# AlerianEmperor/Voxel-Cone-Tracing

Hardware: AMD Instinct MI355X
Metric: Mcones/s (+ ms per GI pass), Sponza-class 256^3 @1080p (higher is better)
Workload: dtype f32; 1 GPU; procedural atrium (Sponza-class, 257488 tris, seed 1234), 256^3 RGBA8 brick chain, 1920x1080, 6 diffuse + 1 specular cone/px, trace of a resident (GPU-rasterised) G-buffer; voxel_dim=256, width=1920, height=1080, cones_per_pixel=7, bounces=1, anisotropic_mips=False, parallelism=single GPU, trace_variant=0, footprint_records=False, comm_reserved_cus=0, raster_form=direct

## Files before the change

### voxel-cone-tracing_amd/csrc/vct_trace.hip

```cpp
#include <hip/hip_fp16.h>

#include <type_traits>

#include "../../include/vct.h"
#include "vct_internal.h"
#include "vct_texel.h"
#include "vct_tilediv.h"


namespace {

struct F3 { float x, y, z; };
struct F4 { float x, y, z, w; };

__device__ __forceinline__ F3 f3(float x, float y, float z) { return {x, y, z}; }
__device__ __forceinline__ float dot3(F3 a, F3 b) { return a.x * b.x + a.y * b.y + a.z * b.z; }
__device__ __forceinline__ F3 cross3(F3 a, F3 b) {
    return {a.y * b.z - a.z * b.y, a.z * b.x - a.x * b.z, a.x * b.y - a.y * b.x};
}
__device__ __forceinline__ float div_rn(float a, float b) { return a / b; }
__device__ __forceinline__ float sqrt_rn(float a) { return __builtin_sqrtf(a); }
__device__ __forceinline__ F3 normalize3(F3 a) {
    const float l = sqrt_rn(dot3(a, a));
    return {div_rn(a.x, l), div_rn(a.y, l), div_rn(a.z, l)};
// ... 71 lines not shown
struct Footprint { int i0, j0, k0; float a, b, c; };
__device__ __forceinline__ Footprint footprint_of(const VctLevelRef lv, float ux, float uy, float uz) {
    const float fN = lv.fN;
    const float u = fmaf(ux, fN, -0.5f), v = fmaf(uy, fN, -0.5f), w = fmaf(uz, fN, -0.5f);
    const float fu = floorf(u), fv = floorf(v), fw = floorf(w);
    const float a = u - fu, b = v - fv, c = w - fw;
    return {(int)fu, (int)fv, (int)fw, a, b, c};
}
struct Anchor { int x, y, z; };
__device__ __forceinline__ int anchor_lane(unsigned long long am) {
    return ((am >> 27) & 1ull) ? 27 : (int)__ffsll((long long)am) - 1;
}
__device__ __forceinline__ Anchor anchor_of(const Footprint& f, int src) {
    return {__builtin_amdgcn_readlane(f.i0, src) - 1, __builtin_amdgcn_readlane(f.j0, src) - 1,
            __builtin_amdgcn_readlane(f.k0, src) - 1};
}
struct BlockFit { int dx, dy, dz; unsigned long long out; };
__device__ __forceinline__ BlockFit block_fit(const Footprint& f, const Anchor an, unsigned long long am) {
    const int dx = f.i0 - an.x, dy = f.j0 - an.y, dz = f.k0 - an.z;
    const uint32_t far = max(max((uint32_t)dx, (uint32_t)dy), (uint32_t)dz);
    return {dx, dy, dz, ballot64(far > 2u) & am};
}
template <bool WRAP>
__device__ __forceinline__ uint32_t block_texel_index(const VctLevelRef lv, const Anchor an, const LaneBlock& lb) {
    if (WRAP) {
        const uint32_t MX = lv.mask_x, MY = MX << 1, MZ = MX << 2;
        const uint32_t m4 = (uint32_t)lv.m << 2;
        const uint32_t sax = spread_byte(lb.lut, an.x, m4) >> 2;
        const uint32_t say = spread_byte(lb.lut, an.y, m4) >> 1;
        const uint32_t saz = spread_byte(lb.lut, an.z, m4);
        return (((sax | ~MX) + lb.sbx) & MX) | (((say | ~MY) + lb.sby) & MY) | (((saz | ~MZ) + lb.sbz) & MZ);
    } else {
        const int x = min(max(an.x + (lb.lane & 3), 0), lv.m);
        const int y = min(max(an.y + ((lb.lane >> 2) & 3), 0), lv.m);
        const int z = min(max(an.z + (lb.lane >> 4), 0), lv.m);
        return vct_morton3((uint32_t)x, (uint32_t)y, (uint32_t)z);
    }
}
__device__ __forceinline__ int block_slot(bool act, int dx, int dy, int dz) { return act ? (dz * 4 + dy) * 4 + dx : 0; }
__device__ __forceinline__ unsigned long long block_texel_mask(const float4 d) {
    return ballot64((__float_as_uint(d.x) | __float_as_uint(d.y) | __float_as_uint(d.z) | __float_as_uint(d.w)) != 0u);
}

#ifndef VCT_REUSE
#define VCT_REUSE 1
#endif
#define VCT_NO_BLOCK 0xfffffff0u
struct BlockDesc {
    uint32_t id;
    Anchor an;
};
__device__ __forceinline__ BlockDesc no_block() { return {VCT_NO_BLOCK, {0, 0, 0}}; }

__device__ __forceinline__ F4 gather_block(const float4* q, float a, float b, float c) {
    F4 r;
    const float a0 = 1.0f - a, b0 = 1.0f - b, c0 = 1.0f - c;
    const float ab00 = a0 * b0, ab10 = a * b0, ab01 = a0 * b, ab11 = a * b;
    {
        const float4 t0 = q[0], t1 = q[1], t2 = q[4], t3 = q[5];
        const float w0 = ab00 * c0, w1 = ab10 * c0, w2 = ab01 * c0, w3 = ab11 * c0;
#define VCT_ACC(ch) r.ch = w0 * t0.ch; r.ch = fmaf(w1, t1.ch, r.ch); r.ch = fmaf(w2, t2.ch, r.ch); r.ch = fmaf(w3, t3.ch, r.ch);
        VCT_ACC(x) VCT_ACC(y) VCT_ACC(z) VCT_ACC(w)
#undef VCT_ACC
    }
    __builtin_amdgcn_sched_barrier(0);
    {
        const float4 t4 = q[16], t5 = q[17], t6 = q[20], t7 = q[21];
        wave_sync();
        const float w4 = ab00 * c, w5 = ab10 * c, w6 = ab01 * c, w7 = ab11 * c;
#define VCT_ACC(ch) r.ch = fmaf(w4, t4.ch, r.ch); r.ch = fmaf(w5, t5.ch, r.ch); r.ch = fmaf(w6, t6.ch, r.ch); r.ch = fmaf(w7, t7.ch, r.ch);
        VCT_ACC(x) VCT_ACC(y) VCT_ACC(z) VCT_ACC(w)
#undef VCT_ACC
    }
    return r;
}

__device__ __forceinline__ void per_lane_census(MarchStats& ms, const Footprint& f, bool act, unsigned long long am, int lane) {
    const int i0 = f.i0, j0 = f.j0, k0 = f.k0;
    ++ms.fallback; ms.fallback_lanes += (uint32_t)__popcll(am);
    int lo[3] = {act ? i0 : 0x7fffffff, act ? j0 : 0x7fffffff, act ? k0 : 0x7fffffff};
    int hi[3] = {act ? i0 : -0x7fffffff, act ? j0 : -0x7fffffff, act ? k0 : -0x7fffffff};
    for (int off = 32; off > 0; off >>= 1)
        for (int q = 0; q < 3; ++q) { lo[q] = min(lo[q], __shfl_xor(lo[q], off)); hi[q] = max(hi[q], __shfl_xor(hi[q], off)); }
    if (hi[0] - lo[0] <= 2 && hi[1] - lo[1] <= 2 && hi[2] - lo[2] <= 2) ++ms.fallback_fits;
    unsigned long long pending = am;
    int nb = 0;
    while (pending != 0ull && nb < 16) {
        const BlockFit fit = block_fit(f, anchor_of(f, (int)__ffsll((long long)pending) - 1), ~0ull);
        pending &= fit.out;
        ++nb;
    }
    int qlo[3] = {act ? i0 : 0x7fffffff, act ? j0 : 0x7fffffff, act ? k0 : 0x7fffffff};
    int qhi[3] = {act ? i0 : -0x7fffffff, act ? j0 : -0x7fffffff, act ? k0 : -0x7fffffff};
    bool qany = act;
    auto widen = [&](int off) {
        for (int q = 0; q < 3; ++q) { qlo[q] = min(qlo[q], __shfl_xor(qlo[q], off)); qhi[q] = max(qhi[q], __shfl_xor(qhi[q], off)); }
        qany = qany || (__shfl_xor((int)qany, off) != 0);
    };
    widen(1); widen(8);
    const int span2 = max(max(qhi[0] - qlo[0], qhi[1] - qlo[1]), qhi[2] - qlo[2]);
    const bool lead2 = (lane & 9) == 0;
    ms.quads_live += (uint32_t)__popcll(ballot64(lead2 && qany));
    ms.quads_fit333 += (uint32_t)__popcll(ballot64(lead2 && qany && span2 <= 1));
    ms.quads_same += (uint32_t)__popcll(ballot64(lead2 && qany && span2 == 0));
    widen(2); widen(16);
    const int span4 = max(max(qhi[0] - qlo[0], qhi[1] - qlo[1]), qhi[2] - qlo[2]);
    const bool lead4 = (lane & 27) == 0;
    ms.quadrants_live += (uint32_t)__popcll(ballot64(lead4 && qany));
    ms.quadrants_fit444 += (uint32_t)__popcll(ballot64(lead4 && qany && span4 <= 2));
    ms.greedy_blocks += (uint32_t)nb;
    if (nb <= 2) ++ms.greedy_le2;
    if (nb <= 3) ++ms.greedy_le3;
    if (nb <= 4) ++ms.greedy_le4;
}

template <bool WRAP, bool COOP, bool LOOSE = false, bool CELLS = false, bool PRIO = false>
__device__ __forceinline__ F4 sample_level(const uint32_t* __restrict__ chain, const VctLevelRef lv,
                                           float ux, float uy, float uz, bool act, unsigned long long am,
                                           float4* __restrict__ blk, const LaneBlock& lb, MarchStats& ms,
                                           const char* __restrict__ cells = nullptr) {
    if (PRIO) __builtin_amdgcn_s_setprio(1);
    const int m = lv.m;
    const Footprint f = footprint_of(lv, ux, uy, uz);
    const float a = f.a, b = f.b, c = f.c;
    const int i0 = f.i0, j0 = f.j0, k0 = f.k0;
    const uint32_t* __restrict__ base = chain + lv.off;
    const uint32_t MX = lv.mask_x, MY = MX << 1, MZ = MX << 2;
    const vct_v4i32 tb = level_texel_buffer(base);

    F4 r = {0.0f, 0.0f, 0.0f, 0.0f};
    const Anchor an = anchor_of(f, anchor_lane(am));
    const BlockFit fit = block_fit(f, an, am);
    if (COOP && fit.out == 0ull) {
        const float4 d = texel_f32(tb, block_texel_index<WRAP>(lv, an, lb));
        if (PRIO) __builtin_amdgcn_s_setprio(0);
        const bool any_texel = block_texel_mask(d) != 0ull;
        if (VCT_STATS) { if (any_texel) ++ms.coop_hit; else ++ms.coop_zero; }
        if (any_texel) {
            blk[lb.lane] = d;
            wave_sync();
            r = gather_block(blk + block_slot(act, fit.dx, fit.dy, fit.dz), a, b, c);
        }
    } else {
      if (VCT_STATS) per_lane_census(ms, f, act, am, lb.lane);
      if (act) {
        uint32_t mx0, mx1, my0, my1, mz0, mz1;
        if (WRAP) {
            if (!CELLS) {
                const uint32_t m4 = (uint32_t)m << 2;
                const char* lutb = (const char*)lb.lut_vec;
                mx0 = *(const uint32_t*)(lutb + (((uint32_t)i0 << 2) & m4)) >> 2;
                my0 = *(const uint32_t*)(lutb + (((uint32_t)j0 << 2) & m4)) >> 1;
                mz0 = *(const uint32_t*)(lutb + (((uint32_t)k0 << 2) & m4));
            } else {
                mx0 = vct_spread3((uint32_t)i0 & (uint32_t)m);
                my0 = vct_spread3((uint32_t)j0 & (uint32_t)m) << 1;
                mz0 = vct_spread3((uint32_t)k0 & (uint32_t)m) << 2;
            }
            mx1 = ((mx0 | ~MX) + 1u) & MX;
            my1 = ((my0 | ~MY) + 2u) & MY;
            mz1 = ((mz0 | ~MZ) + 4u) & MZ;
        } else {
            const int ci0 = min(max(i0, 0), m), ci1 = min(max(i0 + 1, 0), m);
            const int cj0 = min(max(j0, 0), m), cj1 = min(max(j0 + 1, 0), m);
            const int ck0 = min(max(k0, 0), m), ck1 = min(max(k0 + 1, 0), m);
            mx0 = vct_spread3((uint32_t)ci0); mx1 = vct_spread3((uint32_t)ci1);
            my0 = vct_spread3((uint32_t)cj0) << 1; my1 = vct_spread3((uint32_t)cj1) << 1;
            mz0 = vct_spread3((uint32_t)ck0) << 2; mz1 = vct_spread3((uint32_t)ck1) << 2;
        }
        if (!CELLS) {
            const float a0 = 1.0f - a, b0 = 1.0f - b, c0 = 1.0f - c;
            const float ab00 = a0 * b0, ab10 = a * b0, ab01 = a0 * b, ab11 = a * b;
            {
                const float4 f0 = texel_f32(tb, mx0 | my0 | mz0), f1 = texel_f32(tb, mx1 | my0 | mz0);
                const float w0 = ab00 * c0, w1 = ab10 * c0;
#define VCT_ACC(ch) r.ch = w0 * f0.ch; r.ch = fmaf(w1, f1.ch, r.ch);
                VCT_ACC(x) VCT_ACC(y) VCT_ACC(z) VCT_ACC(w)
#undef VCT_ACC
            }
            __builtin_amdgcn_sched_barrier(0);
            {
                const float4 f2 = texel_f32(tb, mx0 | my1 | mz0), f3 = texel_f32(tb, mx1 | my1 | mz0);
                const float w2 = ab01 * c0, w3 = ab11 * c0;
#define VCT_ACC(ch) r.ch = fmaf(w2, f2.ch, r.ch); r.ch = fmaf(w3, f3.ch, r.ch);
                VCT_ACC(x) VCT_ACC(y) VCT_ACC(z) VCT_ACC(w)
#undef VCT_ACC
            }
            __builtin_amdgcn_sched_barrier(0);
            {
                const float4 f4 = texel_f32(tb, mx0 | my0 | mz1), f5 = texel_f32(tb, mx1 | my0 | mz1);
                const float4 f6 = texel_f32(tb, mx0 | my1 | mz1), f7 = texel_f32(tb, mx1 | my1 | mz1);
                if (PRIO) __builtin_amdgcn_s_setprio(0);
                const float w4 = ab00 * c, w5 = ab10 * c, w6 = ab01 * c, w7 = ab11 * c;
#define VCT_ACC(ch) r.ch = fmaf(w4, f4.ch, r.ch); r.ch = fmaf(w5, f5.ch, r.ch); r.ch = fmaf(w6, f6.ch, r.ch); r.ch = fmaf(w7, f7.ch, r.ch);
                VCT_ACC(x) VCT_ACC(y) VCT_ACC(z) VCT_ACC(w)
#undef VCT_ACC
            }
        } else {
            uint32_t t[8];
            if (WRAP && lv.off != 0u) {
                const char* cb = cells + ((size_t)lv.off << 5);
                const uint32_t ro = (mx0 | my0 | mz0) << 5;
                const uint4 lo = *(const uint4*)(cb + ro);
                const uint4 hi = *(const uint4*)(cb + ro + 16u);
                t[0] = lo.x; t[1] = lo.y; t[2] = lo.z; t[3] = lo.w;
                t[4] = hi.x; t[5] = hi.y; t[6] = hi.z; t[7] = hi.w;
            } else {
                t[0] = base[mx0 | my0 | mz0]; t[1] = base[mx1 | my0 | mz0];
                t[2] = base[mx0 | my1 | mz0]; t[3] = base[mx1 | my1 | mz0];
                t[4] = base[mx0 | my0 | mz1]; t[5] = base[mx1 | my0 | mz1];
                t[6] = base[mx0 | my1 | mz1]; t[7] = base[mx1 | my1 | mz1];
            }
            if (PRIO) __builtin_amdgcn_s_setprio(0);
            const float a0 = 1.0f - a, b0 = 1.0f - b, c0 = 1.0f - c;
            const float wg[8] = {(a0 * b0) * c0, (a * b0) * c0, (a0 * b) * c0, (a * b) * c0,
                                 (a0 * b0) * c,  (a * b0) * c,  (a0 * b) * c,  (a * b) * c};
            r.x = wg[0] * unorm8_of<0, LOOSE>(t[0]);
            r.y = wg[0] * unorm8_of<8, LOOSE>(t[0]);
            r.z = wg[0] * unorm8_of<16, LOOSE>(t[0]);
            r.w = wg[0] * unorm8_of<24, LOOSE>(t[0]);
#pragma unroll
            for (int i = 1; i < 8; ++i) {
                r.x = fmaf(wg[i], unorm8_of<0, LOOSE>(t[i]), r.x);
                r.y = fmaf(wg[i], unorm8_of<8, LOOSE>(t[i]), r.y);
                r.z = fmaf(wg[i], unorm8_of<16, LOOSE>(t[i]), r.z);
                r.w = fmaf(wg[i], unorm8_of<24, LOOSE>(t[i]), r.w);
            }
        }
      }
    }
    return r;
}

template <bool WRAP, bool LOOSE, bool PRIO, int SLAB>
__device__ __forceinline__ F4 sample_level_reuse(const uint32_t* __restrict__ chain, const VctLevelRef lv,
                                                 float ux, float uy, float uz, bool act, unsigned long long am,
                                                 float4* __restrict__ blk, const LaneBlock& lb, MarchStats& ms,
                                                 BlockDesc& held) {
    if (PRIO) __builtin_amdgcn_s_setprio(1);
    const Footprint f = footprint_of(lv, ux, uy, uz);
    int mode = 0, at = 0;
    if ((held.id & ~1u) == lv.off) {
        const BlockDesc cd = held;
        const BlockFit fit = block_fit(f, cd.an, am);
        if (VCT_STATS) {
            const Anchor fresh = anchor_of(f, anchor_lane(am));
            ++ms.reuse[SLAB][0];
            if (fit.out == 0ull) { ++ms.reuse[SLAB][1]; if (!(cd.id & 1u)) ++ms.reuse[SLAB][2]; }
            if (fresh.x == cd.an.x && fresh.y == cd.an.y && fresh.z == cd.an.z) ++ms.reuse[SLAB][3];
        }
        if (fit.out == 0ull) {
            if (PRIO) __builtin_amdgcn_s_setprio(0);
            mode = 1 + (int)(cd.id & 1u);
            at = block_slot(act, fit.dx, fit.dy, fit.dz) + 64;
        }
    }
    if (mode == 0) {
        const Anchor an = anchor_of(f, anchor_lane(am));
        const BlockFit fit = block_fit(f, an, am);
        if (fit.out == 0ull) {
            const uint32_t idx = block_texel_index<true>(lv, an, lb);
            const float4 d = texel_f32(level_texel_buffer(chain + lv.off), idx);
            if (PRIO) __builtin_amdgcn_s_setprio(0);
            const unsigned long long any_texel = block_texel_mask(d);
            if (VCT_STATS) { if (any_texel != 0ull) ++ms.coop_hit; else ++ms.coop_zero; }
            mode = any_texel != 0ull ? 2 : 1;
            if (SLAB == 1) held = {lv.off | (uint32_t)(mode - 1), an};
            if (mode == 2) {
                blk[SLAB * 64 + lb.lane] = d;
                wave_sync();
                at = block_slot(act, fit.dx, fit.dy, fit.dz) + SLAB * 64;
            }
        }
    }
    if (mode == 2) return gather_block(blk + at, f.a, f.b, f.c);
    if (mode == 1) return {0.0f, 0.0f, 0.0f, 0.0f};
    return sample_level<WRAP, false, LOOSE, false, PRIO>(chain, lv, ux, uy, uz, act, am, blk, lb, ms);
}

template <bool WRAP, bool COOP, bool LOOSE, bool CELLS, bool PRIO, bool REUSE, int SLAB>
__device__ __forceinline__ F4 sample_step_level(const VctTraceParams& p, const VctLevelRef lv, float ux, float uy, float uz,
                                                bool act, unsigned long long am, float4* __restrict__ blk,
                                                const LaneBlock& lb, MarchStats& ms, BlockDesc& held) {
    if constexpr (REUSE) {
        static_assert(WRAP && COOP && !CELLS, "block reuse: cooperative sampler, GL_REPEAT, no footprint records");
        return sample_level_reuse<WRAP, LOOSE, PRIO, SLAB>(p.chain, lv, ux, uy, uz, act, am, blk, lb, ms, held);
    } else {
        return sample_level<WRAP, COOP, LOOSE, CELLS, PRIO>(p.chain, lv, ux, uy, uz, act, am, blk + SLAB * 64, lb, ms, p.cells_biased);
    }
}

struct AnisoCone {
    float wx, wy, wz;
    bool nx, ny, nz;
};

template <bool WRAP, bool COOP>
__device__ __forceinline__ F4 sample_aniso(const VctTraceParams& p, const VctLevelRef lv, float ux,
                                           float uy, float uz, bool act, unsigned long long m,
                                           float4* __restrict__ blk, const LaneBlock& lb, const AnisoCone& ac,
                                           MarchStats& ms) {
    auto chain_of = [&](int d) { return p.aniso + (size_t)d * p.aniso_stride - p.level_off[1]; };
    const unsigned long long mx = ballot64(ac.nx) & m, my = ballot64(ac.ny) & m, mz = ballot64(ac.nz) & m;
    F4 tx, ty, tz;
    bool done = false;
    if (COOP && WRAP) {
        const Footprint f = footprint_of(lv, ux, uy, uz);
        const Anchor an = anchor_of(f, anchor_lane(m));
        const BlockFit fit = block_fit(f, an, m);
        if (fit.out == 0ull) {
            done = true;
            const uint32_t idx = block_texel_index<true>(lv, an, lb);
            const unsigned long long mneg[3] = {mx, my, mz};
            const bool lneg[3] = {ac.nx, ac.ny, ac.nz};
            uint32_t tpos[3], tneg[3];
#pragma unroll
            for (int k = 0; k < 3; ++k) {
                tpos[k] = mneg[k] != m ? (chain_of(2 * k) + lv.off)[idx] : 0u;
                tneg[k] = mneg[k] != 0ull ? (chain_of(2 * k + 1) + lv.off)[idx] : 0u;
            }
            const int slot = block_slot(act, fit.dx, fit.dy, fit.dz);
            float4* alt = p.aniso_alt_slab ? blk + p.aniso_alt_slab : blk;
            F4 out3[3];
#pragma unroll
            for (int k = 0; k < 3; ++k) {
                F4 r = {0.0f, 0.0f, 0.0f, 0.0f};
                if (ballot64((tpos[k] | tneg[k]) != 0u) != 0ull) {
                    auto dec = [](uint32_t t) {
                        float4 d;
                        d.x = unorm8(t & 0xffu); d.y = unorm8((t >> 8) & 0xffu);
                        d.z = unorm8((t >> 16) & 0xffu); d.w = unorm8(t >> 24);
                        return d;
                    };
                    if (mneg[k] != m) blk[lb.lane] = dec(tpos[k]);
                    if (mneg[k] != 0ull) alt[lb.lane] = dec(tneg[k]);
                    wave_sync();
                    r = gather_block((lneg[k] ? alt : blk) + slot, f.a, f.b, f.c);
                }
                out3[k] = r;
            }
            tx = out3[0]; ty = out3[1]; tz = out3[2];
        }
    }
    if (!done) {
        auto axis_sample = [&](int axis, bool neg, unsigned long long mn) -> F4 {
            if (mn == 0ull) return sample_level<WRAP, COOP>(chain_of(2 * axis), lv, ux, uy, uz, act, m, blk, lb, ms);
            if (mn == m) return sample_level<WRAP, COOP>(chain_of(2 * axis + 1), lv, ux, uy, uz, act, m, blk, lb, ms);
            const F4 a = sample_level<WRAP, COOP>(chain_of(2 * axis), lv, ux, uy, uz, act && !neg, m & ~mn, blk, lb, ms);
            const F4 b = sample_level<WRAP, COOP>(chain_of(2 * axis + 1), lv, ux, uy, uz, act && neg, mn, blk, lb, ms);
            return neg ? b : a;
        };
        tx = axis_sample(0, ac.nx, mx);
        ty = axis_sample(1, ac.ny, my);
        tz = axis_sample(2, ac.nz, mz);
    }
    F4 r;
    r.x = ac.wx * tx.x; r.x = fmaf(ac.wy, ty.x, r.x); r.x = fmaf(ac.wz, tz.x, r.x);
    r.y = ac.wx * tx.y; r.y = fmaf(ac.wy, ty.y, r.y); r.y = fmaf(ac.wz, tz.y, r.y);
    r.z = ac.wx * tx.z; r.z = fmaf(ac.wy, ty.z, r.z); r.z = fmaf(ac.wz, tz.z, r.z);
    r.w = ac.wx * tx.w; r.w = fmaf(ac.wy, ty.w, r.w); r.w = fmaf(ac.wz, tz.w, r.w);
    return r;
}

typedef const __attribute__((address_space(4))) VctStep* StepTable;

__device__ __forceinline__ VctStep load_step(StepTable t, int k) {
    VctStep s;
    s.dist = t[k].dist; s.occ_rcp = t[k].occ_rcp; s.occ_den = t[k].occ_den; s.frac = t[k].frac;
    s.level = t[k].level; s.level2 = t[k].level2; s.two_levels = t[k].two_levels; s.omf = t[k].omf;
    s.l1.off = t[k].l1.off; s.l1.mask_x = t[k].l1.mask_x; s.l1.fN = t[k].l1.fN; s.l1.m = t[k].l1.m;
    s.l2.off = t[k].l2.off; s.l2.mask_x = t[k].l2.mask_x; s.l2.fN = t[k].l2.fN; s.l2.m = t[k].l2.m;
    return s;
}

#define VCT_MARCH_STEP(st, act, live)                                                                        \
        const float px = start.x + dir.x * st.dist; \
        const float py = start.y + dir.y * st.dist; \
        const float pz = start.z + dir.z * st.dist; \
        const float ux = fmaf(div_const<FASTDIV>(px, p.half_G_aux, p.half_G_rcp), 0.5f, 0.5f); \
        const float uy = fmaf(div_const<FASTDIV>(py, p.half_G_aux, p.half_G_rcp), 0.5f, 0.5f); \
        const float uz = fmaf(div_const<FASTDIV>(pz, p.half_G_aux, p.half_G_rcp), 0.5f, 0.5f); \
        F4 vc = (ANISO && st.level >= 1) ? sample_aniso<WRAP, COOP>(p, st.l1, ux, uy, uz, act, live, blk, lb, ac, ms) \
                                         : sample_step_level<WRAP, COOP, FASTDIV == 2, CELLS, PRIO, REUSE, 0>(p, st.l1, ux, uy, uz, act, live, blk, lb, ms, held); \
        if (st.two_levels) { \
            const F4 t2 = ANISO ? sample_aniso<WRAP, COOP>(p, st.l2, ux, uy, uz, act, live, blk + 64, lb, ac, ms) \
                                : sample_step_level<WRAP, COOP, FASTDIV == 2, CELLS, PRIO, REUSE, 1>(p, st.l2, ux, uy, uz, act, live, blk, lb, ms, held); \
            const float g = st.omf;       \
            vc.x = fmaf(st.frac, t2.x, g * vc.x); \
            vc.y = fmaf(st.frac, t2.y, g * vc.y); \
            vc.z = fmaf(st.frac, t2.z, g * vc.z); \
            vc.w = fmaf(st.frac, t2.w, g * vc.w); \
        } \
        if (act) { \
            const float oma = 1.0f - alpha; \
            cr = fmaf(oma, vc.x, cr); \
            cg = fmaf(oma, vc.y, cg); \
            cb = fmaf(oma, vc.z, cb); \
            occ = occ + div_const<FASTDIV>(oma * vc.w, st.occ_den, st.occ_rcp); \
            alpha = fmaf(oma, vc.w, alpha); \
            ++steps; \
        }

typedef const __attribute__((address_space(4))) float* SkyPoly;
__device__ __forceinline__ void sky_epilogue(const VctTraceParams& p, bool alive, F3 d, float alpha, float& cr, float& cg, float& cb) {
    SkyPoly q = (SkyPoly)p.sky;
    float x = d.x, y = d.y, z = d.z;
    asm volatile("" : "+s"(q), "+v"(x), "+v"(y), "+v"(z));
    const float xy = x * y, yz = y * z, zz = fmaf(3.0f * z, z, -1.0f), xz = x * z, xxyy = fmaf(x, x, -(y * y));
    const float T = fmaxf(1.0f - alpha, 0.0f);
    float sky[3];
#pragma unroll
    for (int c = 0; c < 3; ++c) {
        float s = q[c];
        s = fmaf(q[3 + c], y, s);
        s = fmaf(q[6 + c], z, s);
        s = fmaf(q[9 + c], x, s);
        s = fmaf(q[12 + c], xy, s);
        s = fmaf(q[15 + c], yz, s);
        s = fmaf(q[18 + c], zz, s);
        s = fmaf(q[21 + c], xz, s);
        s = fmaf(q[24 + c], xxyy, s);
        sky[c] = fmaxf(s, 0.0f);
    }
    if (alive) {
        cr = fmaf(T, sky[0], cr);
        cg = fmaf(T, sky[1], cg);
        cb = fmaf(T, sky[2], cb);
    }
}

#define VCT_SKY_NONE 0
#define VCT_SKY_INSIDE 1
#define VCT_SKY_ALPHA 2
template <bool WRAP, int FASTDIV, bool COOP, bool ANISO, bool CELLS, bool PRIO, bool REUSE, int SKY = VCT_SKY_NONE>
__device__ __forceinline__ F4 cone_march(const VctTraceParams& p, bool alive, F3 start, F3 dir,
                                         const VctStep* tab_global, int n,
                                         float4* __restrict__ blk, const LaneBlock& lb,
                                         int& steps_out, MarchStats& ms, BlockDesc& held, float* alpha_out = nullptr) {
    const StepTable tab = (StepTable)tab_global;
    float cr = 0.0f, cg = 0.0f, cb = 0.0f, occ = 0.0f;
    int steps = 0;
    AnisoCone ac = {0.0f, 0.0f, 0.0f, false, false, false};
    if (ANISO) {
        ac.wx = dir.x * dir.x; ac.wy = dir.y * dir.y; ac.wz = dir.z * dir.z;
        ac.nx = !(dir.x >= 0.0f); ac.ny = !(dir.y >= 0.0f); ac.nz = !(dir.z >= 0.0f);
    }
    const float wx = start.x + dir.x * p.vs, wy = start.y + dir.y * p.vs, wz = start.z + dir.z * p.vs;
    float alpha = fmaf(wx, 0.0f, fmaf(wy, 0.0f, fmaf(wz, 0.0f, 0.0f)));
    const unsigned long long alive_mask = ballot64(alive);
    if constexpr (!ANISO) {
    auto march_step = [&](const VctStep& st, const bool act, const unsigned long long live) { VCT_MARCH_STEP(st, act, live) };
    VctStep ea = load_step(tab, 0), eb = ea;
    for (int k = 0; k < n;) {
        {
            const bool act = alive && (alpha < p.max_alpha);
            const unsigned long long live = ballot64(alpha < p.max_alpha) & alive_mask;
            if (live == 0ull) break;
            if (VCT_STATS) { ++ms.wave_steps; ms.lane_steps += (uint32_t)__popcll(live); }
            eb = load_step(tab, k + 1 < n ? k + 1 : k);
            march_step(ea, act, live);
            if (++k >= n) break;
        }
        {
            const bool act = alive && (alpha < p.max_alpha);
            const unsigned long long live = ballot64(alpha < p.max_alpha) & alive_mask;
            if (live == 0ull) break;
            if (VCT_STATS) { ++ms.wave_steps; ms.lane_steps += (uint32_t)__popcll(live); }
            ea = load_step(tab, k + 1 < n ? k + 1 : k);
            march_step(eb, act, live);
            ++k;
        }
    }
    } else {
    VctStep nxt = load_step(tab, 0);
    for (int k = 0; k < n; ++k) {
        const bool act = alive && (alpha < p.max_alpha);
        const unsigned long long live = ballot64(alpha < p.max_alpha) & alive_mask;
        if (live == 0ull) break;
        if (VCT_STATS) { ++ms.wave_steps; ms.lane_steps += (uint32_t)__popcll(live); }
        const VctStep st = nxt;
        nxt = load_step(tab, k + 1 < n ? k + 1 : k);
        VCT_MARCH_STEP(st, act, live)
    }
    }
    [[maybe_unused]] const float alpha_seen = steps == 0 ? 0.0f : alpha;
    if (alive && steps == 0 && alpha != alpha && n > 0 && 0.0f < p.max_alpha) {
        cr = cg = cb = occ = __builtin_nanf("");
// ... 200 lines not shown
    const int vb = xcd_remap((int)blockIdx.x, (int)gridDim.x);
    const int ti = vb * VCT_WAVES_PER_BLOCK + wave;
    if (ti >= ntiles) return;

    const LaneBlock lb = make_lane_block(p, lane);
    MarchStats ms = {};

    const int tile = p.tile_row0 * p.tiles_x + ti;
    const int ty = tile_row_of(p, tile), tx = tile - ty * p.tiles_x;
    auto fresh_lane = [&]() { int l = lane; asm volatile("" : "+v"(l)); return l; };
    auto pixel_index = [&]() {
        const int l = fresh_lane();
        return (size_t)(ty * VCT_TILE + (l >> 3)) * p.width + (tx * VCT_TILE + (l & 7));
    };
    auto gbuf_ptr = [&](int l) {
        return p.gbuf + (size_t)tile * (VCT_GB_NPLANES * VCT_TILE_PIX) + l;
    };
    const int x = tx * VCT_TILE + (lane & 7), y = ty * VCT_TILE + (lane >> 3);
    const float* gb = gbuf_ptr(lane);
    const bool in_frame = (x < p.width) && (y < p.height);
    const bool alive = in_frame && !(gb_plane(gb, 18) < 0.5f);

    F3 start, k0, k1, k2;
    cone_frame_from_gbuffer(gb, p.vs, start, k0, k1, k2);

    int total = 0;
    const F4 ind = gather_six_cones(k0, k1, k2, total,
        [&](F3 dir, int& st) { return cone_march<WRAP, FASTDIV, COOP>(p, alive, start, dir, p.steps_diffuse, p.n_diffuse, blk, lb, st, ms); },
        [&](int i, F4 c, int st) { store_debug_cone(p, pixel_index, i, c, st, alive, in_frame); });

    const float* gb2 = gbuf_ptr(fresh_lane());
    const F3 Rd = specular_dir(eye_dir(gb_planes3(gb2, 0), p.cam), gb_planes3(gb2, 12));
    int st6;
    const F4 sc = cone_march<WRAP, FASTDIV, COOP>(p, alive, start, Rd, p.steps_specular, p.n_specular, blk, lb, st6, ms);
    total += st6;
    store_debug_cone(p, pixel_index, 6, sc, st6, alive, in_frame);

    const float* gb3 = gbuf_ptr(fresh_lane());
    if (in_frame) composite<false>(p, gb3, ind, sc, eye_dir(gb_planes3(gb3, 0), p.cam), alive, pixel_index, [] { return (size_t)0; }, p.shininess);
    total = wave_sum(total);
    if (lane == 0) p.tile_steps[tile] = (uint32_t)total;
    flush_stats(p, ms, lane);
}

#ifndef VCT_SPLIT
#define VCT_SPLIT 3
#endif
#define VCT_CONES_PER_WAVE (6 / (VCT_SPLIT - 1))
static_assert(VCT_SPLIT == 3 || VCT_SPLIT == 4 || VCT_SPLIT == 7, "VCT_SPLIT must be 3, 4 or 7");
#ifndef VCT_ANISO_MIN_WAVES
#define VCT_ANISO_MIN_WAVES 5
#endif

typedef const __attribute__((address_space(4))) VctGlossTable* GlossTable;
__device__ __forceinline__ int gloss_class_of(const VctTraceParams& p, int tile, int pix, int nclasses) {
    const int b = (int)p.pix_gloss[(size_t)tile * VCT_TILE_PIX + pix];
    return b < nclasses ? b : 0;
}
template <bool WRAP, int FASTDIV, bool ANISO, bool COMPACT = false, bool CELLS = false, bool PRIO = false, bool COMP = false,
          bool HALF = false, bool GLOSS = false, bool SKY = false>
__global__ void __launch_bounds__(64 * VCT_SPLIT, ANISO ? VCT_ANISO_MIN_WAVES : VCT_TRACE_MIN_WAVES)
k_trace_tile_split(const VctTraceParams p) {
    static_assert(!GLOSS || (COMP && !ANISO && !COMPACT && !CELLS), "gloss classes: the default kernel's COMP forms only");
    static_assert(!SKY || (COMP && !ANISO && !COMPACT && !CELLS), "sky light: the default kernel's COMP forms only");
    __shared__ float4 lds_blk[VCT_SPLIT][ANISO ? 4 : 2][64];
    __shared__ float4 lds_cone[7][64];
    static_assert(64ull * (6 + 8) * VCT_MAX_STEPS < (1ull << 28) && VCT_SPLIT < 16, "the arrival word holds count and step total");
    __shared__ uint32_t lds_arrive;
    const int lane = threadIdx.x & 63;
    const int wave = __builtin_amdgcn_readfirstlane((int)(threadIdx.x >> 6));
    float4* blk = &lds_blk[wave][0][0];
    if (threadIdx.x == 0) lds_arrive = 0u;
    __syncthreads();

    const int ntiles = p.ntiles;
    const int ti = xcd_remap((int)blockIdx.x, (int)gridDim.x);
    if (ti >= ntiles) return;
    constexpr bool compact = COMPACT;
    uint32_t cpix = 0u;
    if (compact) {
        if ((uint32_t)ti >= *p.vt_count) {
            if (threadIdx.x == 0) p.tile_steps[p.tile_row0 * p.tiles_x + ti] = 0u;
            return;
        }
        cpix = p.vt_pix[(size_t)ti * 64 + lane];
    }

    const LaneBlock lb = make_lane_block(p, lane);
    MarchStats ms = {};
    constexpr bool REUSE = VCT_REUSE && WRAP && !ANISO && !CELLS && !COMPACT;
    BlockDesc held = no_block();

    int lrow = 0, tile0 = p.tile_row0 * p.tiles_x + ti;
    if (p.row_stride > 1) {
        lrow = tile_row_of(p, ti);
        tile0 = (p.tile_row0 + lrow * p.row_stride) * p.tiles_x + (ti - lrow * p.tiles_x);
    }
    const bool cvalid = !compact || cpix != 0xffffffffu;
    const int tile = compact ? (cvalid ? (int)(cpix >> 6) : 0) : tile0;
    const int ty = tile_row_of(p, tile), tx = tile - ty * p.tiles_x;
    const int oy = p.pack_rows ? (p.row_stride > 1 ? lrow : ty - p.tile_row0) : ty;
    const int plane_ = compact ? (int)(cpix & 63u) : lane;
    auto fresh_lane = [&]() { int l = plane_; asm volatile("" : "+v"(l)); return l; };
    auto pixel_index = [&]() {
        const int l = fresh_lane();
        return (size_t)(oy * VCT_TILE + (l >> 3)) * p.width + (tx * VCT_TILE + (l & 7));
    };
    auto gbuf_ptr = [&](int l) {
        return p.gbuf + (size_t)tile * (VCT_GB_NPLANES * VCT_TILE_PIX) + l;
    };
    const int x = tx * VCT_TILE + (plane_ & 7), y = ty * VCT_TILE + (plane_ >> 3);
    const float* gb = gbuf_ptr(plane_);
    const bool in_frame = cvalid && (x < p.width) && (y < p.height);
    const bool alive = in_frame && !(gb_plane(gb, 18) < 0.5f);
    int total = 0;
    const uint32_t groups = COMP ? (uint32_t)__builtin_amdgcn_readfirstlane((int)p.comp) >> VCT_COMP_GROUPS_SHIFT : 3u;
    const int n_diffuse = (groups & 1u) ? p.n_diffuse : 0, n_specular = (groups & 2u) ? p.n_specular : 0;
    const bool march_d = SKY ? alive && (groups & 1u) != 0u : alive, march_s = SKY ? alive && (groups & 2u) != 0u : alive;
    if (HALF && wave < VCT_SPLIT - 1) {
    } else if (wave < VCT_SPLIT - 1) {
        F3 start, k0, k1, k2;
        cone_frame_from_gbuffer(gb, p.vs, start, k0, k1, k2);
#pragma unroll 1
        for (int i = wave * VCT_CONES_PER_WAVE; i < wave * VCT_CONES_PER_WAVE + VCT_CONES_PER_WAVE; ++i) {
            int st;
            const F4 c = cone_march<WRAP, FASTDIV, true, ANISO, CELLS, PRIO, REUSE, SKY ? VCT_SKY_INSIDE : VCT_SKY_NONE>(p, march_d, start, cone_dir(k0, k1, k2, i),
                                                                       p.steps_diffuse, n_diffuse, blk, lb, st, ms, held);
            total += st;
            lds_cone[i][lane] = make_float4(c.x, c.y, c.z, c.w);
            store_debug_cone(p, pixel_index, i, c, st, alive, in_frame);
        }
    } else {
        if (!PRIO && p.spec_prio) __builtin_amdgcn_s_setprio(1);
        const F3 P = gb_planes3(gb, 0), Nw = gb_planes3(gb, 3), N = gb_planes3(gb, 12);
        const F3 start = cone_start(P, Nw, p.vs);
        const F3 E = eye_dir(P, p.cam);
        auto hand_over = [&](F3 e) { blk[lane] = make_float4(e.x, e.y, e.z, 0.0f); };
        if constexpr (GLOSS) {
            const GlossTable gt = (GlossTable)p.gloss;
            const int cls = gloss_class_of(p, tile, plane_, gt->nclasses);
            const F3 dir = specular_dir(E, N);
            if (!alive) {
                lds_cone[6][lane] = make_float4(0.0f, 0.0f, 0.0f, 0.0f);
                if (p.dbg_steps && in_frame) p.dbg_steps[pixel_index() * 7 + 6] = 0;
            }
            [[maybe_unused]] float sky_alpha = 0.0f;
            for (unsigned long long rest = ballot64(alive); rest != 0ull;) {
                const int k = __builtin_amdgcn_readlane(cls, (int)__ffsll((long long)rest) - 1);
                const bool mine = alive && cls == k;
                int st;
                float a = 0.0f;
                const F4 sc = cone_march<WRAP, FASTDIV, true, ANISO, CELLS, PRIO, REUSE, SKY ? VCT_SKY_ALPHA : VCT_SKY_NONE>(
                    p, mine && march_s, start, dir, &p.gloss->steps[k][0], (groups & 2u) ? gt->nsteps[k] : 0, blk, lb, st, ms, held, &a);
                total += st;
                if (mine) lds_cone[6][lane] = make_float4(sc.x, sc.y, sc.z, sc.w);
                if (SKY && mine) sky_alpha = a;
                store_debug_cone(p, pixel_index, 6, sc, st, mine && !SKY, mine);
                rest &= ~ballot64(mine);
            }
            if constexpr (SKY) {
                const float4 v = lds_cone[6][lane];
                F4 sc = {v.x, v.y, v.z, v.w};
                sky_epilogue(p, march_s, dir, sky_alpha, sc.x, sc.y, sc.z);
                lds_cone[6][lane] = make_float4(sc.x, sc.y, sc.z, sc.w);
                store_debug_cone(p, pixel_index, 6, sc, 0, alive, false);
            }
            hand_over(eye_dir(gb_planes3(gbuf_ptr(fresh_lane()), 0), p.cam));
        } else {
        int st6;
        const F4 sc = cone_march<WRAP, FASTDIV, true, ANISO, CELLS, PRIO, REUSE, SKY ? VCT_SKY_INSIDE : VCT_SKY_NONE>(p, march_s, start, specular_dir(E, N),
                                                                    p.steps_specular, n_specular, blk, lb, st6, ms, held);
        total += st6;
        lds_cone[6][lane] = make_float4(sc.x, sc.y, sc.z, sc.w);
        store_debug_cone(p, pixel_index, 6, sc, st6, alive, in_frame);
        hand_over(E);
        }
    }
    total = wave_sum(total);
    flush_stats(p, ms, lane, wave == VCT_SPLIT - 1);

    __threadfence_block();
    uint32_t before = 0u;
    if (lane == 0) before = atomicAdd(&lds_arrive, (uint32_t)total + (1u << 28));
    before = (uint32_t)__builtin_amdgcn_readfirstlane((int)before);
    if ((before >> 28) != VCT_SPLIT - 1) return;
    __threadfence_block();
    if (lane == 0) p.tile_steps[tile0] = (before + (uint32_t)total) & 0x0fffffffu;

    const float* gb3 = gbuf_ptr(fresh_lane());
    if (in_frame) {
        F4 ind = {0.0f, 0.0f, 0.0f, 0.0f};
        if (HALF) {
            const float4 v = p.dr_ind[pixel_index()];
            ind = {v.x, v.y, v.z, v.w};
        } else {
#pragma unroll
            for (int i = 0; i < 6; ++i) ind = fold_cone(ind, i, lds_cone[i][lane]);
        }
        float shininess = p.shininess;
        if constexpr (GLOSS) {
            const GlossTable gt = (GlossTable)p.gloss;
            shininess = p.gloss->shininess[gloss_class_of(p, tile, fresh_lane(), gt->nclasses)];
        }
        const float4 e = lds_blk[VCT_SPLIT - 1][0][lane];
        composite<COMP>(p, gb3, ind, lds_cone[6][lane], f3(e.x, e.y, e.z), alive, pixel_index,
                        [&]() { return (size_t)tile * (VCT_EMIS_NPLANES * VCT_TILE_PIX) + fresh_lane(); }, shininess);
    }
}

__device__ __forceinline__ const float* gb_of_pixel(const VctTraceParams& p, int x, int y) {
    return p.gbuf + (size_t)((y >> 3) * p.tiles_x + (x >> 3)) * (VCT_GB_NPLANES * VCT_TILE_PIX) + (((y & 7) << 3) | (x & 7));
}
__device__ __forceinline__ float dot3_rn(F3 a, F3 b) {
    return __fadd_rn(__fadd_rn(__fmul_rn(a.x, b.x), __fmul_rn(a.y, b.y)), __fmul_rn(a.z, b.z));
}
__device__ __forceinline__ uint32_t lane_rank(unsigned long long m) {
    return __builtin_amdgcn_mbcnt_hi((uint32_t)(m >> 32), __builtin_amdgcn_mbcnt_lo((uint32_t)m, 0u));
}

#ifndef VCT_POINT_MIN_WAVES
#define VCT_POINT_MIN_WAVES 5
#endif
template <bool WRAP, int FASTDIV, bool LISTED, int WAVES, bool SKY = false>
__global__ void __launch_bounds__(64 * WAVES, VCT_POINT_MIN_WAVES)
k_point_march(const VctTraceParams p) {
    __shared__ float4 lds_blk[WAVES][2][64];
    __shared__ float4 lds_cone[WAVES == 2 ? 3 : 1][64];
    const int lane = threadIdx.x & 63;
    const int wave = __builtin_amdgcn_readfirstlane((int)(threadIdx.x >> 6));
    float4* blk = &lds_blk[wave][0][0];
    const LaneBlock lb = make_lane_block(p, lane);
    MarchStats ms = {};
    const int cw = (p.width + 1) >> 1, ch = (p.height + 1) >> 1;
    const int bxn = (cw + 7) >> 3;
    const uint32_t nfill = LISTED ? (uint32_t)p.dr_ctr[2 * VCT_DR_COUNTERS] : 0u;
    const uint32_t nitems = LISTED ? (nfill + 63u) >> 6 : (uint32_t)(bxn * ((ch + 7) >> 3));
    unsigned long long wave_steps = 0;
    uint32_t wave_marched = 0u;
    for (uint32_t it = blockIdx.x; it < nitems; it += gridDim.x) {
        int x = 0, y = 0;
        bool alive = false;
        uint32_t code = VCT_DR_NO_ANCHOR;
        const int by = LISTED ? 0 : (int)it / bxn, bx = LISTED ? 0 : (int)it - by * bxn;
        const int cx = bx * 8 + (lane & 7), cy = by * 8 + (lane >> 3);
        if (!LISTED) {
            if (cx < cw && cy < ch) {
#pragma unroll
                for (int k = 0; k < 4; ++k) {
                    const int px = 2 * cx + (k & 1), py = 2 * cy + (k >> 1);
                    if (!alive && px < p.width && py < p.height && !(gb_plane(gb_of_pixel(p, px, py), 18) < 0.5f)) {
                        alive = true; x = px; y = py; code = (uint32_t)k;
                    }
                }
            }
        } else {
            const uint32_t e = it * 64u + (uint32_t)lane;
            if (e < nfill) {
                const uint32_t pix = p.dr_list[e];
// ... 660 lines not shown
```

Baseline: 27790 Mcones/s.

## Raise split-trace occupancy to 8 waves with narrow gathers and trimmed LDS

Adds a NARROW mode that issues trilinear texel and LDS gather loads in pairs with scheduling barriers, which lowers peak register pressure. It raises the launch-bounds minimum waves to 8 for the wrap/cells-or-prio split kernel. LDS use shrinks: wave 0 folds its cones into a running prefix, the last cone of each wave is handed over through its block slab, and the specular result goes through the block buffer rather than a 7x64 float4 cone array. The cost is more serialised load/FMA phases and extra LDS traffic in the cone loop, and spills are possible if 8 waves do not fit the register budget.

Measured after the change: 28340 Mcones/s (median of 6 runs). 2.0% higher.

```diff
diff --git a/voxel-cone-tracing_amd/csrc/vct_trace.hip b/voxel-cone-tracing_amd/csrc/vct_trace.hip
--- a/voxel-cone-tracing_amd/csrc/vct_trace.hip
+++ b/voxel-cone-tracing_amd/csrc/vct_trace.hip
@@ -147,10 +147,46 @@
 };
 __device__ __forceinline__ BlockDesc no_block() { return {VCT_NO_BLOCK, {0, 0, 0}}; }
 
+template <bool NARROW = false>
 __device__ __forceinline__ F4 gather_block(const float4* q, float a, float b, float c) {
     F4 r;
     const float a0 = 1.0f - a, b0 = 1.0f - b, c0 = 1.0f - c;
     const float ab00 = a0 * b0, ab10 = a * b0, ab01 = a0 * b, ab11 = a * b;
+    if constexpr (NARROW) {
+        {
+            const float4 t0 = q[0], t1 = q[1];
+            const float w0 = ab00 * c0, w1 = ab10 * c0;
+#define VCT_ACC(ch) r.ch = w0 * t0.ch; r.ch = fmaf(w1, t1.ch, r.ch);
+            VCT_ACC(x) VCT_ACC(y) VCT_ACC(z) VCT_ACC(w)
+#undef VCT_ACC
+        }
+        __builtin_amdgcn_sched_barrier(0);
+        {
+            const float4 t2 = q[4], t3 = q[5];
+            const float w2 = ab01 * c0, w3 = ab11 * c0;
+#define VCT_ACC(ch) r.ch = fmaf(w2, t2.ch, r.ch); r.ch = fmaf(w3, t3.ch, r.ch);
+            VCT_ACC(x) VCT_ACC(y) VCT_ACC(z) VCT_ACC(w)
+#undef VCT_ACC
+        }
+        __builtin_amdgcn_sched_barrier(0);
+        {
+            const float4 t4 = q[16], t5 = q[17];
+            const float w4 = ab00 * c, w5 = ab10 * c;
+#define VCT_ACC(ch) r.ch = fmaf(w4, t4.ch, r.ch); r.ch = fmaf(w5, t5.ch, r.ch);
+            VCT_ACC(x) VCT_ACC(y) VCT_ACC(z) VCT_ACC(w)
+#undef VCT_ACC
+        }
+        __builtin_amdgcn_sched_barrier(0);
+        {
+            const float4 t6 = q[20], t7 = q[21];
+            wave_sync();
+            const float w6 = ab01 * c, w7 = ab11 * c;
+#define VCT_ACC(ch) r.ch = fmaf(w6, t6.ch, r.ch); r.ch = fmaf(w7, t7.ch, r.ch);
+            VCT_ACC(x) VCT_ACC(y) VCT_ACC(z) VCT_ACC(w)
+#undef VCT_ACC
+        }
+        return r;
+    }
     {
         const float4 t0 = q[0], t1 = q[1], t2 = q[4], t3 = q[5];
         const float w0 = ab00 * c0, w1 = ab10 * c0, w2 = ab01 * c0, w3 = ab11 * c0;
@@ -209,7 +245,7 @@
     if (nb <= 4) ++ms.greedy_le4;
 }
 
-template <bool WRAP, bool COOP, bool LOOSE = false, bool CELLS = false, bool PRIO = false>
+template <bool WRAP, bool COOP, bool LOOSE = false, bool CELLS = false, bool PRIO = false, bool NARROW = false>
 __device__ __forceinline__ F4 sample_level(const uint32_t* __restrict__ chain, const VctLevelRef lv,
                                            float ux, float uy, float uz, bool act, unsigned long long am,
                                            float4* __restrict__ blk, const LaneBlock& lb, MarchStats& ms,
@@ -234,7 +270,7 @@
         if (any_texel) {
             blk[lb.lane] = d;
             wave_sync();
-            r = gather_block(blk + block_slot(act, fit.dx, fit.dy, fit.dz), a, b, c);
+            r = gather_block<NARROW>(blk + block_slot(act, fit.dx, fit.dy, fit.dz), a, b, c);
         }
     } else {
       if (VCT_STATS) per_lane_census(ms, f, act, am, lb.lane);
@@ -282,7 +318,24 @@
 #undef VCT_ACC
             }
             __builtin_amdgcn_sched_barrier(0);
-            {
+            if constexpr (NARROW) {
+                {
+                    const float4 f4 = texel_f32(tb, mx0 | my0 | mz1), f5 = texel_f32(tb, mx1 | my0 | mz1);
+                    const float w4 = ab00 * c, w5 = ab10 * c;
+#define VCT_ACC(ch) r.ch = fmaf(w4, f4.ch, r.ch); r.ch = fmaf(w5, f5.ch, r.ch);
+                    VCT_ACC(x) VCT_ACC(y) VCT_ACC(z) VCT_ACC(w)
+#undef VCT_ACC
+                }
+                __builtin_amdgcn_sched_barrier(0);
+                {
+                    const float4 f6 = texel_f32(tb, mx0 | my1 | mz1), f7 = texel_f32(tb, mx1 | my1 | mz1);
+                    if (PRIO) __builtin_amdgcn_s_setprio(0);
+                    const float w6 = ab01 * c, w7 = ab11 * c;
+#define VCT_ACC(ch) r.ch = fmaf(w6, f6.ch, r.ch); r.ch = fmaf(w7, f7.ch, r.ch);
+                    VCT_ACC(x) VCT_ACC(y) VCT_ACC(z) VCT_ACC(w)
+#undef VCT_ACC
+                }
+            } else {
                 const float4 f4 = texel_f32(tb, mx0 | my0 | mz1), f5 = texel_f32(tb, mx1 | my0 | mz1);
                 const float4 f6 = texel_f32(tb, mx0 | my1 | mz1), f7 = texel_f32(tb, mx1 | my1 | mz1);
                 if (PRIO) __builtin_amdgcn_s_setprio(0);
@@ -327,7 +380,7 @@
     return r;
 }
 
-template <bool WRAP, bool LOOSE, bool PRIO, int SLAB>
+template <bool WRAP, bool LOOSE, bool PRIO, int SLAB, bool NARROW = false>
 __device__ __forceinline__ F4 sample_level_reuse(const uint32_t* __restrict__ chain, const VctLevelRef lv,
                                                  float ux, float uy, float uz, bool act, unsigned long long am,
                                                  float4* __restrict__ blk, const LaneBlock& lb, MarchStats& ms,
@@ -368,20 +421,20 @@
             }
         }
     }
-    if (mode == 2) return gather_block(blk + at, f.a, f.b, f.c);
+    if (mode == 2) return gather_block<NARROW>(blk + at, f.a, f.b, f.c);
     if (mode == 1) return {0.0f, 0.0f, 0.0f, 0.0f};
-    return sample_level<WRAP, false, LOOSE, false, PRIO>(chain, lv, ux, uy, uz, act, am, blk, lb, ms);
-}
-
-template <bool WRAP, bool COOP, bool LOOSE, bool CELLS, bool PRIO, bool REUSE, int SLAB>
+    return sample_level<WRAP, false, LOOSE, false, PRIO, NARROW>(chain, lv, ux, uy, uz, act, am, blk, lb, ms);
+}
+
+template <bool WRAP, bool COOP, bool LOOSE, bool CELLS, bool PRIO, bool REUSE, int SLAB, bool NARROW = false>
 __device__ __forceinline__ F4 sample_step_level(const VctTraceParams& p, const VctLevelRef lv, float ux, float uy, float uz,
                                                 bool act, unsigned long long am, float4* __restrict__ blk,
                                                 const LaneBlock& lb, MarchStats& ms, BlockDesc& held) {
     if constexpr (REUSE) {
         static_assert(WRAP && COOP && !CELLS, "block reuse: cooperative sampler, GL_REPEAT, no footprint records");
-        return sample_level_reuse<WRAP, LOOSE, PRIO, SLAB>(p.chain, lv, ux, uy, uz, act, am, blk, lb, ms, held);
+        return sample_level_reuse<WRAP, LOOSE, PRIO, SLAB, NARROW>(p.chain, lv, ux, uy, uz, act, am, blk, lb, ms, held);
     } else {
-        return sample_level<WRAP, COOP, LOOSE, CELLS, PRIO>(p.chain, lv, ux, uy, uz, act, am, blk + SLAB * 64, lb, ms, p.cells_biased);
+        return sample_level<WRAP, COOP, LOOSE, CELLS, PRIO, NARROW>(p.chain, lv, ux, uy, uz, act, am, blk + SLAB * 64, lb, ms, p.cells_biased);
     }
 }
 
@@ -476,10 +529,10 @@
         const float uy = fmaf(div_const<FASTDIV>(py, p.half_G_aux, p.half_G_rcp), 0.5f, 0.5f); \
         const float uz = fmaf(div_const<FASTDIV>(pz, p.half_G_aux, p.half_G_rcp), 0.5f, 0.5f); \
         F4 vc = (ANISO && st.level >= 1) ? sample_aniso<WRAP, COOP>(p, st.l1, ux, uy, uz, act, live, blk, lb, ac, ms) \
-                                         : sample_step_level<WRAP, COOP, FASTDIV == 2, CELLS, PRIO, REUSE, 0>(p, st.l1, ux, uy, uz, act, live, blk, lb, ms, held); \
+                                         : sample_step_level<WRAP, COOP, FASTDIV == 2, CELLS, PRIO, REUSE, 0, NARROW>(p, st.l1, ux, uy, uz, act, live, blk, lb, ms, held); \
         if (st.two_levels) { \
             const F4 t2 = ANISO ? sample_aniso<WRAP, COOP>(p, st.l2, ux, uy, uz, act, live, blk + 64, lb, ac, ms) \
-                                : sample_step_level<WRAP, COOP, FASTDIV == 2, CELLS, PRIO, REUSE, 1>(p, st.l2, ux, uy, uz, act, live, blk, lb, ms, held); \
+                                : sample_step_level<WRAP, COOP, FASTDIV == 2, CELLS, PRIO, REUSE, 1, NARROW>(p, st.l2, ux, uy, uz, act, live, blk, lb, ms, held); \
             const float g = st.omf;       \
             vc.x = fmaf(st.frac, t2.x, g * vc.x); \
             vc.y = fmaf(st.frac, t2.y, g * vc.y); \
@@ -527,7 +580,7 @@
 #define VCT_SKY_NONE 0
 #define VCT_SKY_INSIDE 1
 #define VCT_SKY_ALPHA 2
-template <bool WRAP, int FASTDIV, bool COOP, bool ANISO, bool CELLS, bool PRIO, bool REUSE, int SKY = VCT_SKY_NONE>
+template <bool WRAP, int FASTDIV, bool COOP, bool ANISO, bool CELLS, bool PRIO, bool REUSE, int SKY = VCT_SKY_NONE, bool NARROW = false>
 __device__ __forceinline__ F4 cone_march(const VctTraceParams& p, bool alive, F3 start, F3 dir,
                                          const VctStep* tab_global, int n,
                                          float4* __restrict__ blk, const LaneBlock& lb,
@@ -834,6 +887,14 @@
 #define VCT_ANISO_MIN_WAVES 5
 #endif
 
+#ifndef VCT_SPLIT_MAX_WAVES
+#define VCT_SPLIT_MAX_WAVES 8
+#endif
+constexpr int split_min_waves(bool wrap, bool aniso, bool compact, bool cells, bool prio, bool half, bool gloss) {
+    if (aniso) return VCT_ANISO_MIN_WAVES;
+    const bool fits = wrap && !compact && !half && (cells || prio);
+    return fits && VCT_SPLIT_MAX_WAVES >= 8 ? 8 : VCT_TRACE_MIN_WAVES;
+}
 typedef const __attribute__((address_space(4))) VctGlossTable* GlossTable;
 __device__ __forceinline__ int gloss_class_of(const VctTraceParams& p, int tile, int pix, int nclasses) {
     const int b = (int)p.pix_gloss[(size_t)tile * VCT_TILE_PIX + pix];
@@ -841,12 +902,18 @@
 }
 template <bool WRAP, int FASTDIV, bool ANISO, bool COMPACT = false, bool CELLS = false, bool PRIO = false, bool COMP = false,
           bool HALF = false, bool GLOSS = false, bool SKY = false>
-__global__ void __launch_bounds__(64 * VCT_SPLIT, ANISO ? VCT_ANISO_MIN_WAVES : VCT_TRACE_MIN_WAVES)
+__global__ void __launch_bounds__(64 * VCT_SPLIT, split_min_waves(WRAP, ANISO, COMPACT, CELLS, PRIO, HALF, GLOSS))
 k_trace_tile_split(const VctTraceParams p) {
+    constexpr bool NARROW = !ANISO && split_min_waves(WRAP, ANISO, COMPACT, CELLS, PRIO, HALF, GLOSS) >= 8;
     static_assert(!GLOSS || (COMP && !ANISO && !COMPACT && !CELLS), "gloss classes: the default kernel's COMP forms only");
     static_assert(!SKY || (COMP && !ANISO && !COMPACT && !CELLS), "sky light: the default kernel's COMP forms only");
     __shared__ float4 lds_blk[VCT_SPLIT][ANISO ? 4 : 2][64];
-    __shared__ float4 lds_cone[7][64];
+    constexpr int RAW_WAVES = VCT_SPLIT - 2, RAW_CONES = VCT_CONES_PER_WAVE - 1;
+    __shared__ float4 lds_raw[RAW_WAVES * RAW_CONES > 0 ? RAW_WAVES * RAW_CONES : 1][64];
+    __shared__ float lds_pre[3][64];
+    __shared__ uint16_t lds_steps[64];
+    __shared__ float4 lds_gloss[GLOSS ? 64 : 1];
+    static_assert(VCT_CONES_PER_WAVE * VCT_MAX_STEPS < (1 << 16), "a lane's steps over the cones of a wave fit lds_steps");
     static_assert(64ull * (6 + 8) * VCT_MAX_STEPS < (1ull << 28) && VCT_SPLIT < 16, "the arrival word holds count and step total");
     __shared__ uint32_t lds_arrive;
     const int lane = threadIdx.x & 63;
@@ -903,27 +970,53 @@
     } else if (wave < VCT_SPLIT - 1) {
         F3 start, k0, k1, k2;
         cone_frame_from_gbuffer(gb, p.vs, start, k0, k1, k2);
+        int carried = 0;
+        const int first = wave * VCT_CONES_PER_WAVE;
+        auto own_lane = [&]() { int l = lane; asm volatile("" : "+v"(l)); return l; };
 #pragma unroll 1
-        for (int i = wave * VCT_CONES_PER_WAVE; i < wave * VCT_CONES_PER_WAVE + VCT_CONES_PER_WAVE; ++i) {
+        for (int i = first; i < first + VCT_CONES_PER_WAVE; ++i) {
             int st;
-            const F4 c = cone_march<WRAP, FASTDIV, true, ANISO, CELLS, PRIO, REUSE, SKY ? VCT_SKY_INSIDE : VCT_SKY_NONE>(p, march_d, start, cone_dir(k0, k1, k2, i),
+            const F4 c = cone_march<WRAP, FASTDIV, true, ANISO, CELLS, PRIO, REUSE, SKY ? VCT_SKY_INSIDE : VCT_SKY_NONE, NARROW>(p, march_d, start, cone_dir(k0, k1, k2, i),
                                                                        p.steps_diffuse, n_diffuse, blk, lb, st, ms, held);
-            total += st;
-            lds_cone[i][lane] = make_float4(c.x, c.y, c.z, c.w);
+            const bool last = i - first == RAW_CONES;
+            const int l = own_lane();
+            F4 out = c;
+            if (wave == 0) {
+                F4 pre = {0.0f, 0.0f, 0.0f, 0.0f};
+                int sum = st;
+                if (i != 0) {
+                    pre = {lds_pre[0][l], lds_pre[1][l], lds_pre[2][l], __int_as_float(carried)};
+                    sum += (int)lds_steps[l];
+                }
+                out = fold_cone(pre, i, c);
+                if (!last) {
+                    lds_pre[0][l] = out.x; lds_pre[1][l] = out.y; lds_pre[2][l] = out.z; carried = __float_as_int(out.w);
+                    lds_steps[l] = (uint16_t)sum;
+                } else carried = sum;
+            } else {
+                carried += st;
+                if (!last) lds_raw[(wave - 1) * RAW_CONES + (i - first)][l] = make_float4(c.x, c.y, c.z, c.w);
+            }
+            if (last) blk[l] = make_float4(out.x, out.y, out.z, out.w);
             store_debug_cone(p, pixel_index, i, c, st, alive, in_frame);
         }
+        total = carried;
     } else {
         if (!PRIO && p.spec_prio) __builtin_amdgcn_s_setprio(1);
         const F3 P = gb_planes3(gb, 0), Nw = gb_planes3(gb, 3), N = gb_planes3(gb, 12);
         const F3 start = cone_start(P, Nw, p.vs);
         const F3 E = eye_dir(P, p.cam);
-        auto hand_over = [&](F3 e) { blk[lane] = make_float4(e.x, e.y, e.z, 0.0f); };
+        auto hand_over_e = [&](F3 e) { blk[lane] = make_float4(e.x, e.y, e.z, 0.0f); };
+        auto hand_over = [&](F4 cone, F3 e) {
+            blk[64 + lane] = make_float4(cone.x, cone.y, cone.z, cone.w);
+            hand_over_e(e);
+        };
         if constexpr (GLOSS) {
             const GlossTable gt = (GlossTable)p.gloss;
             const int cls = gloss_class_of(p, tile, plane_, gt->nclasses);
             const F3 dir = specular_dir(E, N);
             if (!alive) {
-                lds_cone[6][lane] = make_float4(0.0f, 0.0f, 0.0f, 0.0f);
+                lds_gloss[lane] = make_float4(0.0f, 0.0f, 0.0f, 0.0f);
                 if (p.dbg_steps && in_frame) p.dbg_steps[pixel_index() * 7 + 6] = 0;
             }
             [[maybe_unused]] float sky_alpha = 0.0f;
@@ -932,30 +1025,29 @@
                 const bool mine = alive && cls == k;
                 int st;
                 float a = 0.0f;
-                const F4 sc = cone_march<WRAP, FASTDIV, true, ANISO, CELLS, PRIO, REUSE, SKY ? VCT_SKY_ALPHA : VCT_SKY_NONE>(
+                const F4 sc = cone_march<WRAP, FASTDIV, true, ANISO, CELLS, PRIO, REUSE, SKY ? VCT_SKY_ALPHA : VCT_SKY_NONE, NARROW>(
                     p, mine && march_s, start, dir, &p.gloss->steps[k][0], (groups & 2u) ? gt->nsteps[k] : 0, blk, lb, st, ms, held, &a);
                 total += st;
-                if (mine) lds_cone[6][lane] = make_float4(sc.x, sc.y, sc.z, sc.w);
+                if (mine) lds_gloss[lane] = make_float4(sc.x, sc.y, sc.z, sc.w);
                 if (SKY && mine) sky_alpha = a;
                 store_debug_cone(p, pixel_index, 6, sc, st, mine && !SKY, mine);
                 rest &= ~ballot64(mine);
             }
             if constexpr (SKY) {
-                const float4 v = lds_cone[6][lane];
+                const float4 v = lds_gloss[lane];
                 F4 sc = {v.x, v.y, v.z, v.w};
                 sky_epilogue(p, march_s, dir, sky_alpha, sc.x, sc.y, sc.z);
-                lds_cone[6][lane] = make_float4(sc.x, sc.y, sc.z, sc.w);
+                lds_gloss[lane] = make_float4(sc.x, sc.y, sc.z, sc.w);
                 store_debug_cone(p, pixel_index, 6, sc, 0, alive, false);
             }
-            hand_over(eye_dir(gb_planes3(gbuf_ptr(fresh_lane()), 0), p.cam));
+            hand_over_e(eye_dir(gb_planes3(gbuf_ptr(fresh_lane()), 0), p.cam));
         } else {
         int st6;
-        const F4 sc = cone_march<WRAP, FASTDIV, true, ANISO, CELLS, PRIO, REUSE, SKY ? VCT_SKY_INSIDE : VCT_SKY_NONE>(p, march_s, start, specular_dir(E, N),
+        const F4 sc = cone_march<WRAP, FASTDIV, true, ANISO, CELLS, PRIO, REUSE, SKY ? VCT_SKY_INSIDE : VCT_SKY_NONE, NARROW>(p, march_s, start, specular_dir(E, N),
                                                                     p.steps_specular, n_specular, blk, lb, st6, ms, held);
         total += st6;
-        lds_cone[6][lane] = make_float4(sc.x, sc.y, sc.z, sc.w);
         store_debug_cone(p, pixel_index, 6, sc, st6, alive, in_frame);
-        hand_over(E);
+        hand_over(sc, E);
         }
     }
     total = wave_sum(total);
@@ -976,8 +1068,13 @@
             const float4 v = p.dr_ind[pixel_index()];
             ind = {v.x, v.y, v.z, v.w};
         } else {
+            const float4 pre = lds_blk[0][0][lane];
+            ind = {pre.x, pre.y, pre.z, pre.w};
 #pragma unroll
-            for (int i = 0; i < 6; ++i) ind = fold_cone(ind, i, lds_cone[i][lane]);
+            for (int i = VCT_CONES_PER_WAVE; i < 6; ++i) {
+                const int w = i / VCT_CONES_PER_WAVE, j = i % VCT_CONES_PER_WAVE;
+                ind = fold_cone(ind, i, j < RAW_CONES ? lds_raw[(w - 1) * RAW_CONES + j][lane] : lds_blk[w][0][lane]);
+            }
         }
         float shininess = p.shininess;
         if constexpr (GLOSS) {
@@ -985,7 +1082,9 @@
             shininess = p.gloss->shininess[gloss_class_of(p, tile, fresh_lane(), gt->nclasses)];
         }
         const float4 e = lds_blk[VCT_SPLIT - 1][0][lane];
-        composite<COMP>(p, gb3, ind, lds_cone[6][lane], f3(e.x, e.y, e.z), alive, pixel_index,
+        float4 sc;
+        if constexpr (GLOSS) sc = lds_gloss[lane]; else sc = lds_blk[VCT_SPLIT - 1][1][lane];
+        composite<COMP>(p, gb3, ind, sc, f3(e.x, e.y, e.z), alive, pixel_index,
                         [&]() { return (size_t)tile * (VCT_EMIS_NPLANES * VCT_TILE_PIX) + fresh_lane(); }, shininess);
     }
 }
```
